# brech1/keaki

Hardware: AMD Instinct MI355X
Metric: BN254 G1 scalar-mults/sec on 2^24-point MSM (per GPU) (higher is better)
Workload: dtype u32 limbs, 256-bit Montgomery modular integer (9 x 29-bit lazy limbs in the bucket kernel, 8 x 32 elsewhere)

## Files before the change

### keaki_amd/csrc/msm.hip.h

```cpp
#pragma once
#include <type_traits>
#include "bn254_curve.hip.h"
#include "fq29.hip.h"
#include "xyzz29.hip.h"
#include "jac29.hip.h"
#include "xyzz29_g2.hip.h"

namespace bn254 {

typedef uint16_t u16;
typedef u32 v4u_t __attribute__((ext_vector_type(4)));
constexpr u32 DIGIT_NONE = 0xFFFFFFFFu;
#ifndef STAMP
#define STAMP(cond, i) do { } while (0)
#endif

struct MsmShape {
  u32 n;
  u32 c;
  u32 W;
  u32 k;
  u32 stride;
};
KDEV u32 msm_width(const MsmShape& s, u32 w) { return w < s.k ? s.c : s.c - 1; }
// ... 834 lines not shown
    }
    if (threadIdx.x == 0) {
      Xyzz<F> r = sh[0];
      if (mode == HV_ADD) r = xyzz_add(buckets[t], r);
      if constexpr (std::is_same<F, Fq>::value) {
        if (mode == HV_ADD29) {
          U29 X, Y, ZZ, ZZZ;
          if (!acc29_load(state29 + t, X, Y, ZZ, ZZZ)) r = xyzz_add(Xyzz<Fq>{u29_to_fq(X), u29_to_fq(Y), u29_to_fq(ZZ), u29_to_fq(ZZZ)}, r);
        }
        if (mode == HV_SET29 || mode == HV_ADD29)
          acc29_store(state29 + t, u29_from_fq(r.x), u29_from_fq(r.y), u29_from_fq(r.zz), u29_from_fq(r.zzz), xyzz_is_inf(r));
        else
          buckets[t] = r;
      } else {
        buckets[t] = r;
      }
    }
    __syncthreads();
  }
}
KDEV bool msm_bucket_is_heavy(u32 cnt) { return cnt >= HEAVY_MIN; }

template <class F>
__global__ void __launch_bounds__(256) k_msm_accumulate(const Aff<F>* __restrict__ points, SortView v, const u32* __restrict__ counts,
                                                        const u32* __restrict__ perm, u32 nbuckets_total, Xyzz<F>* __restrict__ buckets, u32 cont) {
  u32 lane = blockIdx.x * blockDim.x + threadIdx.x;
  if (lane >= nbuckets_total) return;
  u32 t = perm[lane];
  u32 cnt = counts[t];
  if (msm_bucket_is_heavy(cnt)) return;
  if (cont && cnt == 0) return;
  SegWalker sw;
  seg_init(sw, v, t);
  Xyzz<F> acc = xyzz_inf<F>();
  if (cont) acc = buckets[t];
  for (u32 k = 0; k < cnt; k++) {
    u32 e = seg_next(sw, v);
    Aff<F> p = points[e & 0x7FFFFFFFu];
    acc = xyzz_add_mixed(acc, aff_cneg(p, (e >> 31) != 0));
  }
  buckets[t] = acc;
}

template <int NT>
KDEV Aff<Fq> msm_load_row(const Aff<Fq>* __restrict__ p) {
  if constexpr (NT == 0) {
    return *p;
  } else {
    const v4u_t* s = reinterpret_cast<const v4u_t*>(p);
    const v4u_t w0 = __builtin_nontemporal_load(s), w1 = __builtin_nontemporal_load(s + 1), w2 = __builtin_nontemporal_load(s + 2),
                w3 = __builtin_nontemporal_load(s + 3);
    Aff<Fq> q;
#pragma unroll
    for (int i = 0; i < 4; i++) { q.x.l[i] = w0[i]; q.x.l[4 + i] = w1[i]; q.y.l[i] = w2[i]; q.y.l[4 + i] = w3[i]; }
    return q;
  }
}
#ifdef KEAKI_DIAG
static __global__ void k_diag_mask_rows(u32* __restrict__ sorted, size_t words, u32 mask) {
  for (size_t i = (size_t)blockIdx.x * blockDim.x + threadIdx.x; i < words; i += (size_t)gridDim.x * blockDim.x) {
    const u32 e = sorted[i];
    sorted[i] = (e & 0x80000000u) | (e & mask);
  }
}
#endif
enum { ACC_WHOLE = 0, ACC_FIRST = 1, ACC_MIDDLE = 2, ACC_LAST = 3 };
template <int NT, int MODE, int PF = 2>
static __global__ void __launch_bounds__(256, 3) k_msm_accumulate_g1_u29(const Aff<Fq>* __restrict__ points, SortView v,
                                                                      const u32* __restrict__ counts, const u32* __restrict__ perm,
                                                                      u32 nbuckets_total, Xyzz<Fq>* __restrict__ buckets,
                                                                      Acc29* __restrict__ state29) {
  u32 lane = blockIdx.x * blockDim.x + threadIdx.x;
  if (lane >= nbuckets_total) return;
  u32 t = perm[lane];
  u32 cnt = counts[t];
  if constexpr (MODE == ACC_LAST) {
    if (msm_bucket_is_heavy(cnt)) cnt = 0;
  } else {
    if (msm_bucket_is_heavy(cnt)) return;
  }
  if constexpr (MODE == ACC_MIDDLE) {
    if (cnt == 0) return;
  }
  SegWalker sw;
  SegWalkerQ sq;
  if constexpr (PF != 2) seg_init(sw, v, t);
  U29 X1, Y1, ZZ, ZZZ;
  bool empty = true;
  if constexpr (MODE == ACC_MIDDLE || MODE == ACC_LAST) empty = acc29_load(state29 + t, X1, Y1, ZZ, ZZZ);
  u32 e1 = 0, e2 = 0;
  Aff<Fq> q1;
  __shared__ __attribute__((aligned(16))) u32 idx_slots[PF == 2 ? IDXQ_NQ * IDXQ_PLANE : 4];
  __shared__ __attribute__((aligned(16))) u32 idx_park[PF == 2 ? 256 * SEGQ_PARK : 4];
  const u32* my_slot = idx_slots + threadIdx.x * 4;
  u32* wave_slots = idx_slots + (threadIdx.x & ~63u) * 4;
  u32* park = idx_park + threadIdx.x * SEGQ_PARK;
  if constexpr (PF == 2) {
    segq_init(sq, v, t, park);
    if (cnt > 0) {
      segq_advance(sq, v, t, park);
      segq_fetch(sq, v, wave_slots);
      asm volatile("s_waitcnt vmcnt(0)" ::: "memory");
      e1 = segq_next(sq, v, t, my_slot, wave_slots, park);
      if (cnt > 1) {
        asm volatile("s_waitcnt vmcnt(0)" ::: "memory");
        e2 = segq_next(sq, v, t, my_slot, wave_slots, park);
      }
    }
    q1 = msm_load_row<NT>(points + (e1 & 0x7FFFFFFFu));
  } else if constexpr (PF != 0) {
    e1 = cnt > 0 ? seg_next(sw, v) : 0u; e2 = cnt > 1 ? seg_next(sw, v) : 0u;
    q1 = msm_load_row<NT>(points + (e1 & 0x7FFFFFFFu));
  }
  for (u32 k = 0; k < cnt; k++) {
    u32 e;
    Aff<Fq> q;
    if constexpr (PF == 2) {
      e = e1;
      asm volatile("s_waitcnt vmcnt(0)" ::: "memory");
      q = q1;
#pragma unroll
      for (int i = 0; i < 8; i++) { asm volatile("" : "+v"(q.x.l[i])); asm volatile("" : "+v"(q.y.l[i])); }
      u32 e3 = 0;
      if (k + 2 < cnt) e3 = segq_next(sq, v, t, my_slot, wave_slots, park);
      e1 = e2;
      if (k + 1 < cnt) q1 = msm_load_row<NT>(points + (e1 & 0x7FFFFFFFu));
      e2 = e3;
    } else if constexpr (PF != 0) {
      e = e1;
      q = q1;
      e1 = e2;
      if (k + 1 < cnt) q1 = msm_load_row<NT>(points + (e1 & 0x7FFFFFFFu));
      if (k + 2 < cnt) e2 = seg_next(sw, v);
    } else {
      e = seg_next(sw, v);
      q = msm_load_row<NT>(points + (e & 0x7FFFFFFFu));
    }
    if (aff_is_inf(q)) continue;
    q.y = f_cneg(q.y, (e >> 31) != 0);
    const U29 X2 = u29_from_sat_shift5(q.x.l), Y2 = u29_from_sat_shift5(q.y.l);
    if (empty) {
      X1 = u29_mul(X2, u29_one());
      Y1 = u29_mul(Y2, u29_one());
      ZZ = u29_one();
      ZZZ = u29_one();
      empty = false;
      continue;
    }
    const U29 U2 = u29_mul(X2, ZZ), S2 = u29_mul(Y2, ZZZ);
    const U29 P = u29_sub(U2, X1, Q29::K16), R = u29_sub(S2, Y1, Q29::K4);
    if (u29_maybe_zero(P)) {
      if (u29_is_zero(P)) {
        if (u29_is_zero(R)) {
          Xyzz<Fq> d = xyzz_dbl_aff(q);
          X1 = u29_from_fq(d.x); Y1 = u29_from_fq(d.y); ZZ = u29_from_fq(d.zz); ZZZ = u29_from_fq(d.zzz);
        } else {
          empty = true;
        }
        continue;
      }
    }
    const U29 PP = u29_sqr(P), PPP = u29_mul(P, PP), Q = u29_mul(X1, PP);
    const U29 X3 = u29_sub3(u29_sqr(R), PPP, Q);
    const U29 T = u29_sub(Q, X3, Q29::K16);
    U29 NY1;
#pragma unroll
    for (int i = 0; i < 9; i++) NY1.l[i] = Q29::K2[i] - Y1.l[i];
    Y1 = u29_mul2(R, T, NY1, PPP);
    X1 = X3;
    ZZ = u29_mul(ZZ, PP);
    ZZZ = u29_mul(ZZZ, PPP);
  }
  u32 ts = t;
  asm volatile("" : "+v"(ts));
  if constexpr (MODE == ACC_FIRST || MODE == ACC_MIDDLE) {
    acc29_store(state29 + ts, X1, Y1, ZZ, ZZZ, empty);
  } else {
    Xyzz<Fq> out = xyzz_inf<Fq>();
    if (!empty) {
      out.x = u29_to_fq(X1); out.y = u29_to_fq(Y1); out.zz = u29_to_fq(ZZ); out.zzz = u29_to_fq(ZZZ);
    }
    buckets[ts] = out;
  }
}

template <int CONT>
static __global__ void __launch_bounds__(256, 2) k_msm_accumulate_g2_u29(const Aff<Fq2>* __restrict__ points, SortView v,
                                                                      const u32* __restrict__ counts, const u32* __restrict__ perm,
                                                                      u32 nbuckets_total, Xyzz<Fq2>* __restrict__ buckets) {
  u32 lane = blockIdx.x * blockDim.x + threadIdx.x;
  if (lane >= nbuckets_total) return;
  u32 t = perm[lane];
  u32 cnt = counts[t];
  if (msm_bucket_is_heavy(cnt)) return;
  if (CONT && cnt == 0) return;
  __shared__ __attribute__((aligned(16))) u32 idx_slots[IDXQ_NQ * IDXQ_PLANE];
  __shared__ __attribute__((aligned(16))) u32 idx_park[256 * SEGQ_PARK];
  const u32* my_slot = idx_slots + threadIdx.x * 4;
  u32* wave_slots = idx_slots + (threadIdx.x & ~63u) * 4;
  u32* park = idx_park + threadIdx.x * SEGQ_PARK;
  SegWalkerQ sq;
  segq_init(sq, v, t, park);
  X29G2 acc = x29g2_inf();
  if constexpr (CONT != 0) acc = x29g2_load(buckets[t]);
  if (cnt > 0) {
    segq_advance(sq, v, t, park);
    segq_fetch(sq, v, wave_slots);
  }
  for (u32 k = 0; k < cnt; k++) {
    asm volatile("s_waitcnt vmcnt(0)" ::: "memory");
    const u32 e = segq_next(sq, v, t, my_slot, wave_slots, park);
    Aff<Fq2> q = points[e & 0x7FFFFFFFu];
    x29g2_add_mixed(acc, aff_cneg(q, (e >> 31) != 0));
  }
  u32 ts = t;
  asm volatile("" : "+v"(ts));
  buckets[ts] = x29g2_store(acc);
}

template <class F>
__global__ void __launch_bounds__(64) k_msm_reduce(const Xyzz<F>* __restrict__ buckets, MsmShape s, u32 L, u32 chunks_per_window,
                                                   Xyzz<F>* __restrict__ partials) {
  u32 g = blockIdx.x * blockDim.x + threadIdx.x;
  if (g >= s.W * chunks_per_window) return;
  u32 w = g / chunks_per_window, t = g % chunks_per_window;
  u32 lo = t * L;
  const u32 Bw = msm_nbuckets(s, w);
  const Xyzz<F>* bk = buckets + msm_bucket_base(s, w);
  typedef TailOps<F> O;
  typename O::P run = O::inf(), ws = O::inf();
  for (u32 j = L; j-- > 0;) {
    if (lo + j < Bw) {
      run = O::add(run, O::load(bk[lo + j]));
      ws = O::add(ws, run);
    }
  }
  if (lo != 0 && lo < Bw) {
    typename O::P m = O::inf();
    for (int b = 31 - __clz(lo); b >= 0; b--) {
      m = O::dbl(m);
      if ((lo >> b) & 1) m = O::add(m, run);
    }
    ws = O::add(ws, m);
  }
  partials[g] = O::store(ws);
}

template <class F>
__global__ void __launch_bounds__(64) k_msm_partial_groups(const Xyzz<F>* __restrict__ in, u32 chunks_in, u32 G, u32 chunks_out,
                                                           Xyzz<F>* __restrict__ out) {
  typedef TailOps<F> O;
  __shared__ typename O::P sh[64];
  u32 w = blockIdx.y, x = blockIdx.x, l = threadIdx.x;
  typename O::P acc = O::inf();
  for (u32 t = x * G + l; t < (x + 1) * G && t < chunks_in; t += 64) acc = O::add(acc, O::load(in[(size_t)w * chunks_in + t]));
  sh[l] = acc;
  __syncthreads();
  for (u32 o = 32; o > 0; o >>= 1) {
    if (l < o) sh[l] = O::add(sh[l], sh[l + o]);
    __syncthreads();
  }
  if (l == 0) out[(size_t)w * chunks_out + x] = O::store(sh[0]);
}

template <class F> KDEV void store_norm_jac(F* out, const Xyzz<F>& p);
template <class F>
__global__ void __launch_bounds__(64) k_msm_window_finish(const Xyzz<F>* __restrict__ partials, MsmShape s, u32 chunks_per_window,
                                                          Xyzz<F>* __restrict__ window_sums, F* __restrict__ out_jac) {
  typedef TailOps<F> O;
  __shared__ typename O::P sh[64];
  u32 w = blockIdx.x, l = threadIdx.x;
  typename O::P acc = O::inf();
  for (u32 t = l; t < chunks_per_window; t += 64) acc = O::add(acc, O::load(partials[(size_t)w * chunks_per_window + t]));
  sh[l] = acc;
  __syncthreads();
  for (u32 o = 32; o > 0; o >>= 1) {
    if (l < o) sh[l] = O::add(sh[l], sh[l + o]);
    __syncthreads();
  }
  if (l == 0) {
    typename O::P r = sh[0];
    for (u32 k = 0, nd = msm_bit_offset(s, w); k < nd; k++) r = O::dbl(r);
    if (out_jac) store_norm_jac(out_jac, O::store(r));
    else window_sums[w] = O::store(r);
  }
}

template <class F> KDEV Aff<F> xyzz_to_aff_tail(const Xyzz<F>& p) { return xyzz_to_aff(p); }
template <> KDEV Aff<Fq> xyzz_to_aff_tail<Fq>(const Xyzz<Fq>& p) {
  if (xyzz_is_inf(p)) return aff_inf<Fq>();
  Fq izzz = fq_inv(p.zzz);
  Fq izz = fq_sqr(izzz) * fq_sqr(p.zz);
  return {p.x * izz, p.y * izzz};
}
template <class F>
KDEV void store_norm_jac(F* out, const Xyzz<F>& p) {
  Aff<F> a = xyzz_to_aff_tail(p);
  if (xyzz_is_inf(p)) {
    out[0] = f_one<F>(); out[1] = f_one<F>(); out[2] = f_zero<F>();
  } else {
    out[0] = a.x; out[1] = a.y; out[2] = f_one<F>();
  }
}
template <class F>
__global__ void __launch_bounds__(64) k_msm_final(const Xyzz<F>* __restrict__ window_sums, u32 W, F* __restrict__ out_jac) {
  if (threadIdx.x != 0 || blockIdx.x != 0) return;
  Xyzz<F> acc = xyzz_inf<F>();
  for (u32 w = 0; w < W; w++) acc = xyzz_add(acc, window_sums[w]);
  store_norm_jac(out_jac, acc);
}


template <class F>
__global__ void __launch_bounds__(64) k_msm_build_tables(const Aff<F>* __restrict__ points, u32 N, MsmShape s, Aff<F>* __restrict__ table) {
  u32 i = blockIdx.x * blockDim.x + threadIdx.x;
  if (i >= N) return;
  Aff<F> p = points[i];
  table[i] = p;
#pragma unroll 1
  for (u32 w = 1; w < s.W; w++) {
    Jac<F> j = jac_from_aff(p);
    for (u32 d = msm_width(s, w - 1); d > 0; d--) j = jac_dbl(j);
    p = jac_to_aff(j);
    table[(size_t)w * N + i] = p;
  }
}

constexpr u32 TABLE_MAX_W = 16;
static __global__ void __launch_bounds__(64) k_msm_build_tables_g1(const Aff<Fq>* __restrict__ points, u32 N, MsmShape s, Aff<Fq>* __restrict__ table) {
  u32 i = blockIdx.x * blockDim.x + threadIdx.x;
  if (i >= N) return;
  const Aff<Fq> p = points[i];
  table[i] = p;
  if (aff_is_inf(p)) {
    for (u32 w = 1; w < s.W; w++) table[(size_t)w * N + i] = p;
    return;
  }
  J29 j;
  j.x = u29_from_fq(p.x); j.y = u29_from_fq(p.y); j.z = u29_one();
  U29 zs[TABLE_MAX_W];
  U29 prod = u29_one();
#pragma unroll 1
  for (u32 w = 1; w < s.W; w++) {
    for (u32 d = msm_width(s, w - 1); d > 0; d--) j = j29_dbl(j);
    Aff<Fq> tmp = {u29_to_fq(j.x), u29_to_fq(j.y)};
    table[(size_t)w * N + i] = tmp;
#pragma unroll
    for (u32 k = 1; k < TABLE_MAX_W; k++) if (k == w) zs[k] = j.z;
    prod = u29_mul(prod, j.z);
  }
  U29 tinv = u29_from_fq(fq_inv(u29_to_fq(prod)));
#pragma unroll 1
  for (u32 w = s.W - 1; w >= 1; w--) {
    U29 pre = u29_one(), zw = u29_one();
#pragma unroll
    for (u32 k = 1; k < TABLE_MAX_W; k++) {
      if (k < w) pre = u29_mul(pre, zs[k]);
      if (k == w) zw = zs[k];
    }
    const U29 zinv = u29_mul(tinv, pre);
    tinv = u29_mul(tinv, zw);
    const U29 zi2 = u29_sqr(zinv), zi3 = u29_mul(zi2, zinv);
    const Aff<Fq> jxy = table[(size_t)w * N + i];
    Aff<Fq> a = {u29_to_fq(u29_mul(u29_from_sat_shift5(jxy.x.l), zi2)), u29_to_fq(u29_mul(u29_from_sat_shift5(jxy.y.l), zi3))};
    table[(size_t)w * N + i] = a;
  }
}

template <class F>
__global__ void __launch_bounds__(64) k_sum_jac(const F* __restrict__ pts, u32 k, F* __restrict__ out_jac) {
  if (threadIdx.x != 0 || blockIdx.x != 0) return;
  Xyzz<F> acc = xyzz_inf<F>();
  for (u32 i = 0; i < k; i++) {
    Jac<F> p = {pts[3 * i], pts[3 * i + 1], pts[3 * i + 2]};
    if (jac_is_inf(p)) continue;
    Aff<F> a = f_eq(p.z, f_one<F>()) ? Aff<F>{p.x, p.y} : jac_to_aff(p);
    acc = xyzz_add_mixed(acc, a);
  }
  store_norm_jac(out_jac, acc);
}

}
```

### keaki_amd/csrc/msm_host.hip.h

```cpp
#pragma once
#include <algorithm>
#include <functional>
#include <type_traits>
#include <vector>
#include "internal.h"
#include "msm.hip.h"

namespace keaki_internal {
using namespace bn254;

inline int choose_window(size_t n, int forced = 0) {
  if (forced >= 3 && forced <= 24) return forced;
  if (n < 32) return 3;
  double best = 1e300;
  int bc = 3;
  for (int c = 3; c <= 22; c++) {
    MsmPlan p = msm_make_plan(n, c);
    if (p.nb > ((size_t)PART_MAX_BINS << PART_MAX_FINE_SHIFT)) continue;
    double cost = (double)n * p.s.W + 2.8 * (double)p.nb;
    if ((double)p.nb < 131072.0) cost *= 131072.0 / (double)p.nb;
    if (cost < best) { best = cost; bc = c; }
  }
  return bc;
}

template <class F>
keaki_status msm_dev(keaki_hip_ctx* ctx, const Aff<F>* d_points, size_t srs_len, const void* d_scalars, size_t n, void* d_out_jac,
                     const Aff<F>* d_table = nullptr, int c_table = 0, const MsmPipe* pipe = nullptr) {
  if (!d_out_jac || (n && (!d_points || !d_scalars))) return fail(ctx, KEAKI_ERR_BAD_ARG, "msm: null pointer");
  if (n > srs_len) return fail(ctx, KEAKI_ERR_TOO_LARGE, "msm: %zu scalars but the SRS holds %zu points", n, srs_len);
  if (n >= (1ull << 31)) return fail(ctx, KEAKI_ERR_BAD_ARG, "msm: n must be < 2^31 per device");
  const bool shared = d_table != nullptr && (n * 2 > srs_len || ctx->tune.msm_short_tables != 0);
  const MsmPlan plan = shared ? msm_make_plan(n, c_table) : msm_make_plan(n, choose_window(n, ctx->tune.msm_c));
  MsmShape s = plan.s;
  MsmShape rs = s;
  size_t nb = plan.nb;
  if (shared) {
    s.stride = (u32)srs_len;
    u32 cr = 0;
    while ((1u << cr) < plan.max_b) cr++;
    rs.n = s.n; rs.c = cr; rs.W = 1; rs.k = 1; rs.stride = 0;
    nb = plan.max_b;
    d_points = d_table;
    if ((double)srs_len * s.W >= 2147483647.0) return fail(ctx, KEAKI_ERR_BAD_ARG, "msm: precomputed table index overflows 31 bits");
  }
  ctx->last_c = (int)s.c;
  if ((double)n * s.W >= 4294967295.0) return fail(ctx, KEAKI_ERR_BAD_ARG, "msm: n * windows overflows 32-bit positions");
  u32 L = sizeof(F) > sizeof(Fq) ? (plan.max_b >= 64 ? 8 : plan.max_b)
                                 : plan.max_b >= (1u << 21) ? 32 : plan.max_b >= (1u << 20) ? 16 : (plan.max_b >= 64 ? 8 : plan.max_b);
  if (ctx->tune.reduce_l >= 1 && ctx->tune.reduce_l <= 4096 && (u32)ctx->tune.reduce_l <= plan.max_b) L = (u32)ctx->tune.reduce_l;
  const u32 chunks = cdiv(plan.max_b, L);
  ST_TRY(reserve(ctx, ctx->wsums, (size_t)rs.W * sizeof(Xyzz<F>)));
  Xyzz<F>* wsums = (Xyzz<F>*)ctx->wsums.p;
  F* out = (F*)d_out_jac;
  hipStream_t st = ctx->stream;
  if (ctx->timing) (void)hipEventRecord(ctx->ev[0], st);
  if (n == 0) {
    hipLaunchKernelGGL((k_msm_final<F>), dim3(1), dim3(64), 0, st, (const Xyzz<F>*)wsums, 0u, out);
    return launch_check(ctx, "msm_final");
  }
  const size_t K = pipe ? pipe->ranges.size() : 1;
  if (pipe && K < 1) return fail(ctx, KEAKI_ERR_BAD_ARG, "msm: bad chunk bounds");
  struct Pass {
    size_t lo, m, pairs, max_chunks, cm_bytes, bt_bytes, bm_bytes, sg_bytes, ts_bytes;
    PartShape ps;
  };
  std::vector<Pass> passes(K);
  size_t w_digits = 0, w_sorted = 0, w_offsets = 0, w_cursor = 0, w_pairs = 0, w_total = 0;
  for (size_t j = 0; j < K; j++) {
    Pass& q = passes[j];
    q.lo = pipe ? pipe->ranges[j].first : 0;
    q.m = pipe ? pipe->ranges[j].second : n;
    if (q.m == 0 || q.lo > n || q.m > n - q.lo) return fail(ctx, KEAKI_ERR_BAD_ARG, "msm: bad chunk bounds");
    w_total += q.m;
    if (!part_make_shape(q.m, s.W, nb, &q.ps, ctx->tune.part_shift))
      return fail(ctx, KEAKI_ERR_BAD_ARG, "msm: %zu buckets / %u windows exceed the bucket sort's LDS budget (window too large)", nb, s.W);
    q.pairs = q.m * (size_t)s.W;
    q.max_chunks = part_max_chunks(q.pairs, q.ps.nbins);
    q.cm_bytes = (size_t)q.ps.nbins * q.ps.ntiles * sizeof(uint2);
    q.bt_bytes = ((size_t)q.ps.nbins * 4 + 15) & ~(size_t)15;
    q.bm_bytes = (size_t)q.ps.nbins * sizeof(BinMeta);
    q.sg_bytes = nb * sizeof(v4u_t);
    q.ts_bytes = (size_t)q.ps.ntiles * (q.ps.nbins + 1) * 2;
    w_digits = std::max(w_digits, (size_t)q.ps.ntiles * q.ps.te * 4);
    w_sorted = std::max(w_sorted, q.pairs * 4 + 64);
    w_offsets = std::max(w_offsets, q.max_chunks * q.ps.nf * 4);
    w_cursor = std::max(w_cursor, q.cm_bytes + q.bt_bytes + q.bm_bytes + q.sg_bytes + q.ts_bytes);
    w_pairs = std::max(w_pairs, q.pairs);
  }
  if (w_total != n) return fail(ctx, KEAKI_ERR_BAD_ARG, "msm: the chunks cover %zu of %zu pairs", w_total, n);
  bool u29 = false;
  if constexpr (std::is_same<F, Fq>::value) u29 = ctx->tune.acc_u29;
  if constexpr (std::is_same<F, Fq2>::value) u29 = ctx->tune.acc_u29_g2;
  bool lazy_state = K > 1 && u29 && std::is_same<F, Fq>::value;
  ST_TRY(reserve(ctx, ctx->digits, w_digits));
  ST_TRY(reserve(ctx, ctx->sorted, w_sorted));
  ST_TRY(reserve(ctx, ctx->hist, nb * 4));
  ST_TRY(reserve(ctx, ctx->offsets, w_offsets));
  ST_TRY(reserve(ctx, ctx->cursor, w_cursor));
  ST_TRY(reserve(ctx, ctx->buckets, nb * sizeof(Xyzz<F>)));
  ST_TRY(reserve(ctx, ctx->partials, ((size_t)rs.W * chunks + (size_t)rs.W * 256) * sizeof(Xyzz<F>)));
  ST_TRY(reserve(ctx, ctx->perm, nb * 4 + 2 * CNT_BINS * 4 + sizeof(HeavyList)));
  const u32 hv_cap = (u32)(w_pairs / HEAVY_MIN + 1), hv_slice_cap = (u32)(hv_cap + w_pairs / HEAVY_SLICE + 1);
  const size_t hv_hdr = ((2 * (size_t)hv_cap + hv_slice_cap) * 4 + 255) & ~(size_t)255;
  ST_TRY(reserve(ctx, ctx->heavy, hv_hdr + (size_t)hv_slice_cap * sizeof(Xyzz<F>)));
  if (lazy_state) {
    const keaki_status st29 = reserve(ctx, ctx->acc29, nb * sizeof(Acc29));
    if (st29 == KEAKI_ERR_OOM) { lazy_state = false; u29 = false; ctx->err.clear(); }
    else if (st29 != KEAKI_OK) return st29;
  }
  u32 *tiles = (u32*)ctx->digits.p, *sorted = (u32*)ctx->sorted.p, *hist = (u32*)ctx->hist.p;
  u32* segoff = (u32*)ctx->offsets.p;
  Xyzz<F>* buckets = (Xyzz<F>*)ctx->buckets.p;
  Xyzz<F>* partials = (Xyzz<F>*)ctx->partials.p;
  Acc29* state29 = lazy_state ? (Acc29*)ctx->acc29.p : nullptr;
  u32* perm = (u32*)ctx->perm.p;
  u32 *gstart = perm + nb, *ghist = gstart + CNT_BINS;
  HeavyList* hv = (HeavyList*)(ghist + CNT_BINS);
  u32 *hv_bucket = (u32*)ctx->heavy.p, *hv_first = hv_bucket + hv_cap, *hv_owner = hv_first + hv_cap;
  Xyzz<F>* hv_slices = (Xyzz<F>*)((char*)ctx->heavy.p + hv_hdr);
  for (size_t j = 0; j < K; j++) {
    const Pass& q = passes[j];
    const PartShape& ps = q.ps;
    if (pipe && pipe->stage) ST_TRY(pipe->stage(j));
    MsmShape sj = s;
    sj.n = (u32)q.m;
    const Fr* scal = (const Fr*)d_scalars + q.lo;
    const Aff<F>* pts = d_points + q.lo;
    const bool first = j == 0, last = j + 1 == K;
    uint2* cellmeta = (uint2*)ctx->cursor.p;
    u32* bin_total = (u32*)((char*)ctx->cursor.p + q.cm_bytes);
    BinMeta* bins = (BinMeta*)((char*)bin_total + q.bt_bytes);
    v4u_t* segtab = (v4u_t*)((char*)bins + q.bm_bytes);
    u16* tstart = (u16*)((char*)segtab + q.sg_bytes);
    {
      const dim3 g1(ps.ntiles < ctx->n_cu ? ps.ntiles : ctx->n_cu), b1(T1_THREADS);
#define KEAKI_TILE_SORT(WS) hipLaunchKernelGGL(k_tile_sort<WS>, g1, b1, 0, st, scal, sj, ps, tiles, tstart)
      switch (s.W) {
        case 11: KEAKI_TILE_SORT(11); break;
        case 12: KEAKI_TILE_SORT(12); break;
        case 13: KEAKI_TILE_SORT(13); break;
        case 14: KEAKI_TILE_SORT(14); break;
        case 15: KEAKI_TILE_SORT(15); break;
        case 16: KEAKI_TILE_SORT(16); break;
        default: KEAKI_TILE_SORT(0); break;
      }
#undef KEAKI_TILE_SORT
    }
    ST_TRY(launch_check(ctx, "tile_sort"));
    hipLaunchKernelGGL(k_cell_prefix, dim3(ps.nbins), dim3(1024), 0, st, (const u16*)tstart, ps, cellmeta, bin_total);
    hipLaunchKernelGGL(k_bin_scan, dim3(1), dim3(1024), 0, st, (const u32*)bin_total, ps.nbins, bins);
    {
#define KEAKI_CHUNK_SORT1(L, R, Q, M)                                                                                                                  \
  hipLaunchKernelGGL((k_chunk_sort<L, R, Q, M>), dim3(ps.nbins), dim3(C2_THREADS), 0, st, (const u32*)tiles, (const uint2*)cellmeta, (const BinMeta*)bins, sj, \
                     ps, (u32)nb, sorted, segtab, segoff, hist)
#define KEAKI_CHUNK_SORT(L, R, Q) do { if (ctx->tune.cs_masked) KEAKI_CHUNK_SORT1(L, R, Q, true); else KEAKI_CHUNK_SORT1(L, R, Q, false); } while (0)
      switch (ps.geom) {
        case 0: KEAKI_CHUNK_SORT(8, 1, 16); break;
        case 1: KEAKI_CHUNK_SORT(16, 1, 16); break;
        case 2: KEAKI_CHUNK_SORT(16, 2, 8); break;
        default: KEAKI_CHUNK_SORT(16, 4, 4); break;
      }
#undef KEAKI_CHUNK_SORT1
#undef KEAKI_CHUNK_SORT
    }
    ST_TRY(launch_check(ctx, "chunk_sort"));
#ifdef KEAKI_DIAG
    if (ctx->tune.diag_row_mask) hipLaunchKernelGGL(k_diag_mask_rows, dim3(4096), dim3(256), 0, st, sorted, (size_t)q.pairs, (u32)ctx->tune.diag_row_mask);
#endif
    const SortView view = {sorted, bins, segtab, segoff, ps};
    HIP_TRY(ctx, hipMemsetAsync(ghist, 0, CNT_BINS * 4 + sizeof(HeavyList), st));
    hipLaunchKernelGGL(k_cnt_hist, dim3(cdiv(nb, 1024)), dim3(256), 0, st, (const u32*)hist, (u32)nb, ghist, hv, hv_cap, hv_slice_cap, hv_bucket, hv_first,
                       hv_owner);
    hipLaunchKernelGGL(k_cnt_offsets, dim3(1), dim3(CNT_BINS), 0, st, (const u32*)ghist, gstart);
    hipLaunchKernelGGL(k_cnt_scatter, dim3(cdiv(nb, 1024)), dim3(256), 0, st, (const u32*)hist, (u32)nb, gstart, perm);
    ST_TRY(launch_check(ctx, "cnt_sort"));
    if (ctx->timing && last) (void)hipEventRecord(ctx->ev[1], st);
    const dim3 ga(cdiv(nb, 256)), ba(256);
    bool done = false;
    if constexpr (std::is_same<F, Fq>::value) {
      if (u29) {
#define KEAKI_ACC(NT, MODE) hipLaunchKernelGGL((k_msm_accumulate_g1_u29<NT, MODE>), ga, ba, 0, st, pts, view, (const u32*)hist, (const u32*)perm, (u32)nb, buckets, state29)
        if (K == 1) {
          if (ctx->tune.acc_nt) KEAKI_ACC(1, ACC_WHOLE);
          else if (!ctx->tune.acc_prefetch)
            hipLaunchKernelGGL((k_msm_accumulate_g1_u29<0, ACC_WHOLE, 0>), ga, ba, 0, st, pts, view, (const u32*)hist, (const u32*)perm, (u32)nb, buckets, state29);
          else if (!ctx->tune.acc_idxq)
            hipLaunchKernelGGL((k_msm_accumulate_g1_u29<0, ACC_WHOLE, 1>), ga, ba, 0, st, pts, view, (const u32*)hist, (const u32*)perm, (u32)nb, buckets, state29);
          else KEAKI_ACC(0, ACC_WHOLE);
        }
        else if (first) KEAKI_ACC(0, ACC_FIRST);
        else if (!last) KEAKI_ACC(0, ACC_MIDDLE);
        else KEAKI_ACC(0, ACC_LAST);
#undef KEAKI_ACC
        done = true;
      }
    }
    if constexpr (std::is_same<F, Fq2>::value) {
      if (u29) {
        if (first) hipLaunchKernelGGL(k_msm_accumulate_g2_u29<0>, ga, ba, 0, st, pts, view, (const u32*)hist, (const u32*)perm, (u32)nb, buckets);
        else hipLaunchKernelGGL(k_msm_accumulate_g2_u29<1>, ga, ba, 0, st, pts, view, (const u32*)hist, (const u32*)perm, (u32)nb, buckets);
        done = true;
      }
    }
    if (!done)
      hipLaunchKernelGGL((k_msm_accumulate<F>), ga, ba, 0, st, pts, view, (const u32*)hist, (const u32*)perm, (u32)nb, buckets, first ? 0u : 1u);
    ST_TRY(launch_check(ctx, "msm_accumulate"));
    const u32 hv_mode = lazy_state && !last ? (first ? HV_SET29 : HV_ADD29) : (first ? HV_SET : HV_ADD);
    hipLaunchKernelGGL((k_msm_heavy<F>), dim3(HEAVY_GRID), dim3(256), 0, st, pts, view, (const u32*)hist,
                       (const HeavyList*)hv, hv_slice_cap, (const u32*)hv_bucket, (const u32*)hv_first, (const u32*)hv_owner, hv_slices);
    hipLaunchKernelGGL((k_msm_heavy_combine<F>), dim3(HEAVY_COMBINE_GRID), dim3(64), 0, st, (const u32*)hist, (const HeavyList*)hv, hv_cap, hv_slice_cap,
                       (const u32*)hv_bucket, (const u32*)hv_first, (const Xyzz<F>*)hv_slices, buckets, hv_mode, state29);
    ST_TRY(launch_check(ctx, "msm_heavy"));
  }
  if (ctx->timing) (void)hipEventRecord(ctx->ev[2], st);
  hipLaunchKernelGGL((k_msm_reduce<F>), dim3(cdiv((size_t)rs.W * chunks, 64)), dim3(64), 0, st, (const Xyzz<F>*)buckets, rs, L, chunks, partials);
  const Xyzz<F>* fin_in = partials;
  u32 fin_chunks = chunks;
  if (chunks > 256) {
    const u32 G = cdiv(chunks, 128);
    const u32 chunks2 = cdiv(chunks, G);
    Xyzz<F>* partials2 = partials + (size_t)rs.W * chunks;
    hipLaunchKernelGGL((k_msm_partial_groups<F>), dim3(chunks2, rs.W), dim3(64), 0, st, (const Xyzz<F>*)partials, chunks, G, chunks2, partials2);
    fin_in = partials2; fin_chunks = chunks2;
  }
  hipLaunchKernelGGL((k_msm_window_finish<F>), dim3(rs.W), dim3(64), 0, st, fin_in, rs, fin_chunks, wsums, rs.W == 1 ? out : (F*)nullptr);
  if (rs.W != 1) hipLaunchKernelGGL((k_msm_final<F>), dim3(1), dim3(64), 0, st, (const Xyzz<F>*)wsums, rs.W, out);
  ST_TRY(launch_check(ctx, "msm_reduce/final"));
  if (ctx->timing) {
    (void)hipEventRecord(ctx->ev[3], st);
    ctx->timing_pending = true;
  }
  return KEAKI_OK;
}

template <class F>
keaki_status msm_build_tables(keaki_hip_ctx* ctx, const Aff<F>* d_points, size_t N, int c_table, Aff<F>* d_table) {
  MsmPlan plan = msm_make_plan(N, c_table);
  bool done = false;
  if constexpr (std::is_same<F, Fq>::value) {
    if (plan.s.W <= TABLE_MAX_W) {
      hipLaunchKernelGGL(k_msm_build_tables_g1, dim3(cdiv(N, 64)), dim3(64), 0, ctx->stream, d_points, (u32)N, plan.s, d_table);
      done = true;
    }
  }
  if (!done)
  hipLaunchKernelGGL((k_msm_build_tables<F>), dim3(cdiv(N, 64)), dim3(64), 0, ctx->stream, d_points, (u32)N, plan.s, d_table);
  return launch_check(ctx, "msm_build_tables");
}
inline int choose_window_shared(size_t n, int forced = 0) {
  if (forced >= 3 && forced <= 24) return forced;
  double best = 1e300;
  int bc = 8;
  for (int c = 8; c <= 23; c++) {
    MsmPlan p = msm_make_plan(n, c);
    if (p.max_b > ((size_t)PART_MAX_BINS << PART_MAX_FINE_SHIFT)) continue;
    double cost = (double)n * p.s.W + 2.8 * (double)p.max_b;
    if ((double)p.max_b < 131072.0) cost *= 131072.0 / (double)p.max_b;
    if (cost < best) { best = cost; bc = c; }
  }
  return bc;
}
inline u32 msm_plan_windows(size_t n, int c) { return msm_make_plan(n, c).s.W; }

}
```

Baseline: 1.051 billion.

## Replace running-sum bucket reduction with row/column bit-plane decomposition for shared tables

For the precomputed-table path (single window), the bucket reduction now views the 2^cr buckets as an NR x NC grid. It computes column and row partial sums in tiled kernels, then groups them by index bit into per-bit planes that are doubled and summed. The plain sums replace the sequential running-sum chain, so the reduction becomes additions spread across many workgroups plus a few doublings, instead of long serial chunks followed by weighting. It adds four kernel launches and extra scratch memory, and a benchmark script is included to compare it with the chained reduction.

```diff
diff --git a/bench_tools/sweep_msm_tail.py b/bench_tools/sweep_msm_tail.py
--- /dev/null
+++ b/bench_tools/sweep_msm_tail.py
@@ -0,0 +1,65 @@
+import os, sys, time
+import numpy as np, torch
+sys.path.insert(0, os.path.dirname(os.path.dirname(os.path.abspath(__file__))))
+from keaki_amd.hip import KeakiHip
+from bench import random_fr_limbs
+from oracle import bn254_py as py
+
+REPS = 8
+WIDTHS = {16: (13, 14, 15, 17), 18: (14, 15, 17, 19), 20: (15, 17, 19, 0), 22: (17, 19, 21, 0), 24: (19, 0)}
+
+
+def max_b(c):
+    W = (254 + c - 1) // c
+    base, rem = 254 // W, 254 % W
+    cc, k = (base + 1, rem) if rem else (base, W)
+    widths = [cc if w < k else cc - 1 for w in range(W)]
+    return max([1 << (wd - 1) for wd in widths[:-1]] + [1 << widths[-1]])
+
+
+def old_l(b):
+    return 32 if b >= 1 << 21 else 16 if b >= 1 << 20 else 8
+
+
+def main():
+    limbs = lambda x: np.frombuffer(int(x).to_bytes(32, "little"), np.uint64)
+    g1 = np.concatenate([limbs(py.G1_GEN[0] * (1 << 256) % py.P), limbs(py.G1_GEN[1] * (1 << 256) % py.P)])
+    h = KeakiHip(0)
+    dev = lambda a: torch.from_numpy(np.ascontiguousarray(a).view(np.int64)).cuda()
+    print("# %d MSMs per figure, two rounds chain / rowcol / chain / rowcol, ms per MSM (the faster round)" % REPS)
+    for ln in [int(a) for a in sys.argv[1:]] or sorted(WIDTHS):
+        n = 1 << ln
+        d_gen = dev(g1); d_k = dev(random_fr_limbs(n, 9)); d_pts = torch.empty(n * 8, dtype=torch.int64, device="cuda")
+        h.g1_mul_batch_dev(d_gen.data_ptr(), 0, d_k.data_ptr(), n, d_pts.data_ptr())
+        sc = dev(random_fr_limbs(n, 3))
+        out = torch.empty(12, dtype=torch.int64, device="cuda")
+        for c in WIDTHS[ln]:
+            h.set_option("msm_c_shared", c)
+            srs = h.srs_g1_wrap_dev(d_pts.data_ptr(), n)
+            h.srs_g1_precompute(srs)
+            best, refs = {}, {}
+            for rnd in range(2):
+                for name in ("old", "new"):
+                    h.msm_g1_dev(srs, sc.data_ptr(), n, out.data_ptr()); h.synchronize()
+                    cw = h.last_msm_stats()["window_bits"]
+                    b = max_b(cw)
+                    h.set_option("reduce_l", old_l(b) if name == "old" else 0)
+                    h.msm_g1_dev(srs, sc.data_ptr(), n, out.data_ptr()); h.synchronize()
+                    refs[name] = out.cpu().numpy().copy()
+                    t0 = time.perf_counter()
+                    for _ in range(REPS): h.msm_g1_dev(srs, sc.data_ptr(), n, out.data_ptr())
+                    h.synchronize()
+                    ms = (time.perf_counter() - t0) / REPS * 1e3
+                    best[name] = min(best.get(name, 1e9), ms)
+            h.set_option("reduce_l", 0)
+            same = np.array_equal(refs["old"], refs["new"])
+            print("n=2^%d msm_c_shared=%d window_bits=%d buckets=2^%d  chain(L=%d) %.3f ms  rowcol %.3f ms  %+.3f ms%s"
+                  % (ln, c, cw, b.bit_length() - 1, old_l(b), best["old"], best["new"], best["new"] - best["old"], "" if same else "  RESULTS DIFFER"), flush=True)
+            srs.free()
+        del d_pts, d_k, sc
+        h.trim()
+    h.close()
+
+
+if __name__ == "__main__":
+    main()
diff --git a/keaki_amd/csrc/msm.hip.h b/keaki_amd/csrc/msm.hip.h
--- a/keaki_amd/csrc/msm.hip.h
+++ b/keaki_amd/csrc/msm.hip.h
@@ -1160,6 +1160,100 @@
     out[0] = a.x; out[1] = a.y; out[2] = f_one<F>();
   }
 }
+constexpr u32 ROWCOL_MIN_CR = 12;
+template <class O>
+KDEV typename O::P tail_tree(typename O::P acc, typename O::P* sh, u32 t, u32 n, u32 stop) {
+  for (u32 o = n >> 1; o >= stop; o >>= 1) {
+    if (t >= o && t < 2 * o) sh[t - o] = acc;
+    __syncthreads();
+    if (t < o) acc = O::add(acc, sh[t]);
+    __syncthreads();
+  }
+  return acc;
+}
+template <class F> struct RowColOcc { static constexpr int WGS = 1; };
+template <> struct RowColOcc<Fq> { static constexpr int WGS = 3; };
+
+template <class F>
+__global__ void __launch_bounds__(256, RowColOcc<F>::WGS) k_msm_rowcol(const Xyzz<F>* __restrict__ buckets, u32 cr, Xyzz<F>* __restrict__ colp,
+                                                                      Xyzz<F>* __restrict__ rowp) {
+  typedef TailOps<F> O;
+  __shared__ typename O::P sh[128];
+  const u32 k = (cr + 1) >> 1, NC = 1u << k, ntc = NC >> 6, tiles = 1u << (cr - 12);
+  const u32 g = tiles >= 8 ? 8u : 1u, x = blockIdx.x;
+  const u32 type = (x / g) & 1u, tile = (x / (2 * g)) * g + x % g;
+  const u32 tr = tile / ntc, tc = tile % ntc;
+  const u32 t = threadIdx.x, a = t & 63u, q = t >> 6;
+  const Xyzz<F>* p = type == 0 ? buckets + ((size_t)(tr * 64 + q * 16) << k) + tc * 64 + a : buckets + ((size_t)(tr * 64 + a) << k) + tc * 64 + q;
+  const size_t step = type == 0 ? NC : 4;
+  typename O::P acc = O::inf();
+#pragma unroll 1
+  for (u32 i = 0; i < 16; i++) acc = O::add(acc, O::load(p[i * step]));
+  acc = tail_tree<O>(acc, sh, t, 256, 64);
+  if (t < 64) {
+    if (type == 0) colp[(size_t)tr * NC + tc * 64 + a] = O::store(acc);
+    else rowp[(size_t)(tr * 64 + a) * ntc + tc] = O::store(acc);
+  }
+}
+
+template <class F>
+__global__ void __launch_bounds__(256) k_msm_rowcol_sums(const Xyzz<F>* __restrict__ colp, const Xyzz<F>* __restrict__ rowp, u32 cr,
+                                                         Xyzz<F>* __restrict__ sums) {
+  typedef TailOps<F> O;
+  __shared__ typename O::P sh[128];
+  const u32 k = (cr + 1) >> 1, NC = 1u << k, NR = 1u << (cr - k), ntc = NC >> 6, ntr = NR >> 6;
+  const u32 t = threadIdx.x, a = t & 31u, q = t >> 5;
+  const u32 o = blockIdx.x * 32 + a;
+  const bool col = o < NC;
+  const Xyzz<F>* p = col ? colp + o : rowp + (size_t)(o - NC) * ntc;
+  const u32 terms = col ? ntr : ntc;
+  const size_t step = col ? NC : 1;
+  typename O::P acc = O::inf();
+#pragma unroll 1
+  for (u32 i = q; i < terms; i += 8) acc = O::add(acc, O::load(p[i * step]));
+  acc = tail_tree<O>(acc, sh, t, 256, 32);
+  if (t < 32) sums[o] = O::store(acc);
+}
+
+template <class F>
+__global__ void __launch_bounds__(256) k_msm_rowcol_planes(const Xyzz<F>* __restrict__ sums, u32 cr, Xyzz<F>* __restrict__ planes) {
+  typedef TailOps<F> O;
+  __shared__ typename O::P sh[128];
+  const u32 k = (cr + 1) >> 1, NC = 1u << k, NR = 1u << (cr - k);
+  const u32 t = threadIdx.x, pl = blockIdx.x;
+  typename O::P acc = O::inf();
+  u32 nd = k;
+  if (pl == k) {
+    if (t == 0) acc = O::load(sums[NC - 1]);
+  } else {
+    const bool col = pl < k;
+    const u32 j = col ? pl : pl - k - 1, half = (col ? NC : NR) >> 1;
+    const u32 base = col ? 0u : NC + 1u;
+    nd = col ? j : j + k;
+#pragma unroll 1
+    for (u32 m = t; m < half; m += 256) {
+      const u32 v = ((m >> j) << (j + 1)) | (1u << j) | (m & ((1u << j) - 1u));
+      acc = O::add(acc, O::load(sums[base + v - 1u]));
+    }
+  }
+  acc = tail_tree<O>(acc, sh, t, 256, 1);
+  if (t == 0) {
+    for (u32 d = 0; d < nd; d++) acc = O::dbl(acc);
+    planes[pl] = O::store(acc);
+  }
+}
+
+template <class F>
+__global__ void __launch_bounds__(64) k_msm_rowcol_final(const Xyzz<F>* __restrict__ planes, u32 np, F* __restrict__ out_jac) {
+  typedef TailOps<F> O;
+  __shared__ typename O::P sh[32];
+  const u32 t = threadIdx.x;
+  typename O::P acc = O::inf();
+  if (t < np) acc = O::load(planes[t]);
+  acc = tail_tree<O>(acc, sh, t, 64, 1);
+  if (t == 0) store_norm_jac(out_jac, O::store(acc));
+}
+
 template <class F>
 __global__ void __launch_bounds__(64) k_msm_final(const Xyzz<F>* __restrict__ window_sums, u32 W, F* __restrict__ out_jac) {
   if (threadIdx.x != 0 || blockIdx.x != 0) return;
diff --git a/keaki_amd/csrc/msm_host.hip.h b/keaki_amd/csrc/msm_host.hip.h
--- a/keaki_amd/csrc/msm_host.hip.h
+++ b/keaki_amd/csrc/msm_host.hip.h
@@ -23,6 +23,9 @@
   }
   return bc;
 }
+
+constexpr u32 ROWCOL_MIN_B = 1u << 12;
+static_assert(ROWCOL_MIN_B >= (1u << ROWCOL_MIN_CR), "k_msm_rowcol needs one 64 x 64 tile");
 
 template <class F>
 keaki_status msm_dev(keaki_hip_ctx* ctx, const Aff<F>* d_points, size_t srs_len, const void* d_scalars, size_t n, void* d_out_jac,
@@ -50,6 +53,8 @@
                                  : plan.max_b >= (1u << 21) ? 32 : plan.max_b >= (1u << 20) ? 16 : (plan.max_b >= 64 ? 8 : plan.max_b);
   if (ctx->tune.reduce_l >= 1 && ctx->tune.reduce_l <= 4096 && (u32)ctx->tune.reduce_l <= plan.max_b) L = (u32)ctx->tune.reduce_l;
   const u32 chunks = cdiv(plan.max_b, L);
+  const bool rowcol = ctx->tune.reduce_l == 0 && rs.W == 1 && plan.max_b >= ROWCOL_MIN_B;
+  const size_t rc_points = rowcol ? (size_t)plan.max_b / 32 + 2 * ((size_t)1 << ((rs.c + 1) / 2)) + 32 : 0;
   ST_TRY(reserve(ctx, ctx->wsums, (size_t)rs.W * sizeof(Xyzz<F>)));
   Xyzz<F>* wsums = (Xyzz<F>*)ctx->wsums.p;
   F* out = (F*)d_out_jac;
@@ -99,7 +104,7 @@
   ST_TRY(reserve(ctx, ctx->offsets, w_offsets));
   ST_TRY(reserve(ctx, ctx->cursor, w_cursor));
   ST_TRY(reserve(ctx, ctx->buckets, nb * sizeof(Xyzz<F>)));
-  ST_TRY(reserve(ctx, ctx->partials, ((size_t)rs.W * chunks + (size_t)rs.W * 256) * sizeof(Xyzz<F>)));
+  ST_TRY(reserve(ctx, ctx->partials, std::max((size_t)rs.W * chunks + (size_t)rs.W * 256, rc_points) * sizeof(Xyzz<F>)));
   ST_TRY(reserve(ctx, ctx->perm, nb * 4 + 2 * CNT_BINS * 4 + sizeof(HeavyList)));
   const u32 hv_cap = (u32)(w_pairs / HEAVY_MIN + 1), hv_slice_cap = (u32)(hv_cap + w_pairs / HEAVY_SLICE + 1);
   const size_t hv_hdr = ((2 * (size_t)hv_cap + hv_slice_cap) * 4 + 255) & ~(size_t)255;
@@ -214,18 +219,27 @@
     ST_TRY(launch_check(ctx, "msm_heavy"));
   }
   if (ctx->timing) (void)hipEventRecord(ctx->ev[2], st);
-  hipLaunchKernelGGL((k_msm_reduce<F>), dim3(cdiv((size_t)rs.W * chunks, 64)), dim3(64), 0, st, (const Xyzz<F>*)buckets, rs, L, chunks, partials);
-  const Xyzz<F>* fin_in = partials;
-  u32 fin_chunks = chunks;
-  if (chunks > 256) {
-    const u32 G = cdiv(chunks, 128);
-    const u32 chunks2 = cdiv(chunks, G);
-    Xyzz<F>* partials2 = partials + (size_t)rs.W * chunks;
-    hipLaunchKernelGGL((k_msm_partial_groups<F>), dim3(chunks2, rs.W), dim3(64), 0, st, (const Xyzz<F>*)partials, chunks, G, chunks2, partials2);
-    fin_in = partials2; fin_chunks = chunks2;
-  }
-  hipLaunchKernelGGL((k_msm_window_finish<F>), dim3(rs.W), dim3(64), 0, st, fin_in, rs, fin_chunks, wsums, rs.W == 1 ? out : (F*)nullptr);
-  if (rs.W != 1) hipLaunchKernelGGL((k_msm_final<F>), dim3(1), dim3(64), 0, st, (const Xyzz<F>*)wsums, rs.W, out);
+  if (rowcol) {
+    const u32 cr = rs.c, kc = (cr + 1) / 2, NC = 1u << kc, NR = 1u << (cr - kc);
+    Xyzz<F>*colp = partials, *rowp = colp + (size_t)(NR / 64) * NC, *sums = rowp + (size_t)NR * (NC / 64), *planes = sums + NC + NR;
+    hipLaunchKernelGGL((k_msm_rowcol<F>), dim3(2u << (cr - 12)), dim3(256), 0, st, (const Xyzz<F>*)buckets, cr, colp, rowp);
+    hipLaunchKernelGGL((k_msm_rowcol_sums<F>), dim3((NC + NR) / 32), dim3(256), 0, st, (const Xyzz<F>*)colp, (const Xyzz<F>*)rowp, cr, sums);
+    hipLaunchKernelGGL((k_msm_rowcol_planes<F>), dim3(cr + 1), dim3(256), 0, st, (const Xyzz<F>*)sums, cr, planes);
+    hipLaunchKernelGGL((k_msm_rowcol_final<F>), dim3(1), dim3(64), 0, st, (const Xyzz<F>*)planes, cr + 1, out);
+  } else {
+    hipLaunchKernelGGL((k_msm_reduce<F>), dim3(cdiv((size_t)rs.W * chunks, 64)), dim3(64), 0, st, (const Xyzz<F>*)buckets, rs, L, chunks, partials);
+    const Xyzz<F>* fin_in = partials;
+    u32 fin_chunks = chunks;
+    if (chunks > 256) {
+      const u32 G = cdiv(chunks, 128);
+      const u32 chunks2 = cdiv(chunks, G);
+      Xyzz<F>* partials2 = partials + (size_t)rs.W * chunks;
+      hipLaunchKernelGGL((k_msm_partial_groups<F>), dim3(chunks2, rs.W), dim3(64), 0, st, (const Xyzz<F>*)partials, chunks, G, chunks2, partials2);
+      fin_in = partials2; fin_chunks = chunks2;
+    }
+    hipLaunchKernelGGL((k_msm_window_finish<F>), dim3(rs.W), dim3(64), 0, st, fin_in, rs, fin_chunks, wsums, rs.W == 1 ? out : (F*)nullptr);
+    if (rs.W != 1) hipLaunchKernelGGL((k_msm_final<F>), dim3(1), dim3(64), 0, st, (const Xyzz<F>*)wsums, rs.W, out);
+  }
   ST_TRY(launch_check(ctx, "msm_reduce/final"));
   if (ctx->timing) {
     (void)hipEventRecord(ctx->ev[3], st);
```

Result: faster. 1.062 billion, median of 6 (+1.1%).
